# seung-lab/crackle

Measured on AMD Instinct MI355X. Metric: voxels/s encode+decode, 1024x1024x512 uint32; bit-exact .ckl bytes, higher is better.
Workload: dtype u32

## Files before the change

crackle_amd/csrc/ckl_trail.hpp:

```cpp
#pragma once

#include "ckl_device.hpp"

namespace ckl {
namespace dev {

constexpr uint32_t kTrailTileShift = 5, kTrailTileDim = 32;
__device__ __forceinline__ uint32_t mt_index(uint32_t mx, uint32_t my, uint32_t mtx2) {
	return (((my >> 1) * mtx2 + (mx >> 1)) << 2) | ((my & 1u) << 1) | (mx & 1u);
}
struct MicroTile {
	uint4 lo, hi;
	uint32_t mx, my;
	__device__ __forceinline__ bool holds(uint32_t x, uint32_t y) const { return (x >> 3) == mx && (y >> 3) == my; }
	__device__ __forceinline__ uint32_t nib(uint32_t x, uint32_t y) const {
		const uint32_t r = y & 7u;
		const uint32_t a0 = (r & 1u) ? lo.y : lo.x, a1 = (r & 1u) ? lo.w : lo.z, a2 = (r & 1u) ? hi.y : hi.x, a3 = (r & 1u) ? hi.w : hi.z;
		const uint32_t b0 = (r & 2u) ? a1 : a0, b1 = (r & 2u) ? a3 : a2;
		return (((r & 4u) ? b1 : b0) >> ((x & 7u) * 4u)) & 15u;
	}
};

enum : uint32_t { TRAIL_ERR_CAPACITY = 1u };
constexpr uint32_t kDartNone = 0xFFFFFFFFu;
// ... 532 lines not shown
			val = cm_load(j);
			if (val != ~0ull) {
				root = tuf_find<LDS>(parent, j);
				if (root == j) root = 0xFFFFFFFFu;
			}
		}
		unsigned long long todo = __ballot(root != 0xFFFFFFFFu);
		while (todo) {
			const int first = __ffsll(static_cast<long long>(todo)) - 1;
			const uint32_t r0 = __shfl(root, first, kWave);
			const bool mine = (root == r0);
			unsigned long long v = mine ? val : ~0ull;
#pragma unroll
			for (int s = kWave / 2; s >= 1; s >>= 1) {
				const unsigned long long o = __shfl_xor(v, s, kWave);
				v = o < v ? o : v;
			}
			if ((threadIdx.x & (kWave - 1)) == first) atomicMin(compmin + r0, v);
			todo &= ~__ballot(mine);
		}
	}
	__syncthreads();
	if (!CMLDS) __threadfence();
	stamp(13);
	uint32_t* bits = a.start_bits + static_cast<uint64_t>(zi) * a.start_words;
	for (uint32_t j = threadIdx.x; j < nn; j += kCompBlock) {
		if (tuf_load<LDS>(parent, j) != j) continue;
		const unsigned long long m = cm_load(j);
		if (m == ~0ull) continue;
		const uint32_t minv = static_cast<uint32_t>(m >> 32);
		const uint32_t d = static_cast<uint32_t>(m);
		const uint64_t db = nb * 4u;
		const uint32_t len = a.dart_len[db + d];
		const uint32_t mp = a.dart_minpos[db + d];
		const uint32_t d2 = a.dart_end[db + d];
		atomicOr(bits + (minv >> 5), 1u << (minv & 31u));
		{
			const uint32_t slot = atomicAdd(s_nstart, 1u);
			if (slot < kStartList) start_tmp[slot] = minv;
		}
		const uint32_t pos = mp >> 2, arr = mp & 3u;
		if (pos == 0 || pos == len) continue;
		const uint32_t s = atomicAdd(a.n_nodes + zi, 1u);
		if (s >= a.ncap[zi]) { atomicOr(a.slice_err + zi, TRAIL_ERR_CAPACITY); continue; }
		a.node_vertex[nb + s] = minv;
		a.node_adj[nb + s] = 5u;
		a.vert2node[static_cast<uint64_t>(zi) * a.nverts + minv] = s;
		const uint32_t other = arr ^ 2u;
		for (uint32_t q = 0; q < 4; q++) { a.dart_end[db + s * 4u + q] = kDartNone; a.dart_len[db + s * 4u + q] = 0; a.dart_inline[db + s * 4u + q] = 0; }
		a.dart_end[db + d] = (s << 2) | arr;        a.dart_len[db + d] = pos;
		a.dart_end[db + d2] = (s << 2) | other;     a.dart_len[db + d2] = len - pos;
		a.dart_end[db + s * 4u + arr] = d;          a.dart_len[db + s * 4u + arr] = pos;
		a.dart_end[db + s * 4u + other] = d2;       a.dart_len[db + s * 4u + other] = len - pos;
	}
	__syncthreads();
	if (LDS && CMLDS) __threadfence_block(); else __threadfence();
	stamp(14);
	uint32_t* starts = a.starts + nb;
	const uint32_t cap = a.kcap[zi];
	const uint32_t n_listed = *s_nstart;
	if (n_listed <= kStartList) {
		for (uint32_t i = threadIdx.x; i < n_listed; i += kCompBlock) {
			const uint32_t v = __hip_atomic_load(start_tmp + i, __ATOMIC_RELAXED, __HIP_MEMORY_SCOPE_AGENT);
			uint32_t rank = 0;
			for (uint32_t q = 0; q < n_listed; q++) rank += __hip_atomic_load(start_tmp + q, __ATOMIC_RELAXED, __HIP_MEMORY_SCOPE_AGENT) < v ? 1u : 0u;
			if (rank < cap) starts[rank] = v;
			else atomicOr(a.slice_err + zi, TRAIL_ERR_CAPACITY);
		}
		if (threadIdx.x == 0) a.n_starts[zi] = n_listed < cap ? n_listed : cap;
		stamp(15);
		return;
	}
	constexpr uint32_t kPer = 8;
	uint32_t carry = 0, err = 0;
	for (uint32_t w0 = 0; w0 < a.start_words; w0 += kCompBlock * kPer) {
		uint32_t b[kPer], cnt = 0;
#pragma unroll
		for (uint32_t q = 0; q < kPer; q++) {
			const uint32_t wi = w0 + threadIdx.x * kPer + q;
			b[q] = wi < a.start_words ? __hip_atomic_load(bits + wi, __ATOMIC_RELAXED, __HIP_MEMORY_SCOPE_AGENT) : 0u;
			cnt += __popc(b[q]);
		}
		uint32_t v[1] = { cnt }, tot[1];
		block_excl_add<1, kCompBlock / kWave>(v, tot, s_scan);
		uint32_t o = carry + v[0];
#pragma unroll
		for (uint32_t q = 0; q < kPer; q++) {
			const uint32_t wi = w0 + threadIdx.x * kPer + q;
			for (uint32_t m = b[q]; m; m &= m - 1u) {
				if (o < cap) starts[o] = wi * 32u + (__ffs(m) - 1);
				else err = TRAIL_ERR_CAPACITY;
				o++;
			}
		}
		carry += tot[0];
	}
	if (threadIdx.x == 0) a.n_starts[zi] = carry < cap ? carry : cap;
	if (err) atomicOr(a.slice_err + zi, err);
	stamp(15);
}

static __global__ void __launch_bounds__(kCompBlock) k_trail_components(TrailArgs a, uint32_t lds_bytes) {
	extern __shared__ unsigned long long s_comp[];
	__shared__ uint32_t s_scan[kCompBlock / kWave];
	__shared__ uint32_t s_nstart;
	const uint32_t zi = blockIdx.x + a.z0;
	const uint32_t nn = min(a.n_nodes[zi], a.ncap[zi]);
	if (threadIdx.x == 0) s_nstart = 0;
	__syncthreads();
	if (static_cast<uint64_t>(nn) * 12u <= lds_bytes) trail_components_slice<true, true>(a, zi, reinterpret_cast<uint32_t*>(s_comp + nn), s_comp, nn, s_scan, &s_nstart);
	else if (static_cast<uint64_t>(nn) * 4u <= lds_bytes) trail_components_slice<true, false>(a, zi, reinterpret_cast<uint32_t*>(s_comp), a.compmin + a.nbase[zi], nn, s_scan, &s_nstart);
	else trail_components_slice<false, false>(a, zi, a.parent + a.nbase[zi], a.compmin + a.nbase[zi], nn, s_scan, &s_nstart);
}

enum : uint32_t { TCODE_UP = 0, TCODE_RIGHT = 1, TCODE_DOWN = 2, TCODE_LEFT = 3, TCODE_NONE = 0xFE };

struct TrailTabLds {
	uint8_t* adj;
	unsigned long long* end4;
	__device__ __forceinline__ void load(uint32_t j, uint32_t& av, uint32_t& e_lo, uint32_t& e_hi) const {
		const uint32_t a0 = adj[j];
		const unsigned long long e = end4[j];
		av = __builtin_amdgcn_readfirstlane(a0);
		e_lo = __builtin_amdgcn_readfirstlane(static_cast<uint32_t>(e));
		e_hi = __builtin_amdgcn_readfirstlane(static_cast<uint32_t>(e >> 32));
	}
	__device__ __forceinline__ uint32_t pick(uint32_t e_lo, uint32_t e_hi, uint32_t k) const {
		const uint32_t w = (k & 2u) ? e_hi : e_lo;
		return (w >> ((k & 1u) * 16u)) & 0xFFFFu;
	}
	__device__ __forceinline__ void set_adj(uint32_t j, uint32_t v) const { adj[j] = static_cast<uint8_t>(v); }
};
struct TrailTabGlobal {
	uint8_t* adj;
	const uint32_t* end;
	__device__ __forceinline__ void load(uint32_t j, uint32_t& av, uint32_t& e_lo, uint32_t& e_hi) const {
		const uint32_t* w = reinterpret_cast<const uint32_t*>(reinterpret_cast<uintptr_t>(adj + j) & ~static_cast<uintptr_t>(3));
		const uint32_t sh = static_cast<uint32_t>(reinterpret_cast<uintptr_t>(adj + j) & 3u) * 8u;
		av = (__builtin_amdgcn_readfirstlane(__hip_atomic_load(w, __ATOMIC_RELAXED, __HIP_MEMORY_SCOPE_AGENT)) >> sh) & 0xFFu;
		e_lo = j; e_hi = 0;
	}
	__device__ __forceinline__ uint32_t pick(uint32_t e_lo, uint32_t e_hi, uint32_t k) const { return __builtin_amdgcn_readfirstlane(end[e_lo * 4u + k]); }
	__device__ __forceinline__ void set_adj(uint32_t j, uint32_t v) const {
		uint32_t* w = reinterpret_cast<uint32_t*>(reinterpret_cast<uintptr_t>(adj + j) & ~static_cast<uintptr_t>(3));
		const uint32_t sh = static_cast<uint32_t>(reinterpret_cast<uintptr_t>(adj + j) & 3u) * 8u;
		const uint32_t old = __hip_atomic_load(w, __ATOMIC_RELAXED, __HIP_MEMORY_SCOPE_AGENT);
		__hip_atomic_store(w, (old & ~(0xFFu << sh)) | ((v & 0xFFu) << sh), __ATOMIC_RELAXED, __HIP_MEMORY_SCOPE_AGENT);
	}
};

constexpr uint32_t kEvSeg = 0u << 30, kEvBseg = 1u << 30, kEvDead = 2u << 30, kEvEnd = 3u << 30, kEvMask = 3u << 30;
constexpr uint32_t kEvFormatAddr12 = 1u << 31;
constexpr uint32_t kEvWalkWide = 1u << 30;

template <typename TAB>
__device__ __forceinline__ void trail_walk_slice(
	const TrailArgs& a, uint32_t zi, const TAB& tab, uint2* s_stack2, uint32_t lds_slots
) {
	const uint64_t nb = a.nbase[zi];
	const uint32_t* starts = a.starts + nb;
	const uint32_t n_starts = a.n_starts[zi];
	uint32_t* ev = a.events + a.ibase[zi];
	const uint32_t ecap = a.icap[zi];
	uint32_t* st_node = a.stack_node + a.sbase[zi];
	uint32_t* st_ev = a.stack_item + a.sbase[zi];
	const uint32_t scap = a.scap[zi];
	uint32_t* ch_node = a.chain_node + a.kbase[zi];
	uint32_t* ch_ev0 = a.chain_ev0 + a.kbase[zi];
	const uint32_t kcap = a.kcap[zi];
	const uint32_t* vert2node = a.vert2node + static_cast<uint64_t>(zi) * a.nverts;
	const uint32_t cap1 = lds_slots - 1u;

	uint32_t ne = 0, nch = 0, err = 0;
	const unsigned long long dbg_t0 = (kTuning && a.dbg) ? __builtin_amdgcn_s_memtime() : 0ull;
	const unsigned long long dbg_r0 = (kTuning && a.dbg) ? __builtin_amdgcn_s_memrealtime() : 0ull;
	for (uint32_t si = 0; si < n_starts && !err; si++) {
		const uint32_t sv = __builtin_amdgcn_readfirstlane(starts[si]);
		uint32_t j = __builtin_amdgcn_readfirstlane(vert2node[sv]);
		if (nch < kcap) { ch_node[nch] = sv; ch_ev0[nch] = ne; }
		else err |= TRAIL_ERR_CAPACITY;
		nch++;
		uint32_t sp = 0, pend = 0;
		for (;;) {
			if (ne + 2u > ecap) { err |= TRAIL_ERR_CAPACITY; break; }
			uint32_t av_raw, e_lo, e_hi;
			tab.load(j, av_raw, e_lo, e_hi);
			const uint2 top = s_stack2[sp < cap1 ? sp : cap1];
			const uint32_t av = av_raw & ~pend;
			if (av == 0) {
				tab.set_adj(j, 0u);
				if (sp == 0) { ev[ne] = kEvEnd; ne++; break; }
				uint32_t pj = __builtin_amdgcn_readfirstlane(top.x), pev = __builtin_amdgcn_readfirstlane(top.y);
				if (sp > cap1) {
					pj = __builtin_amdgcn_readfirstlane(__hip_atomic_load(st_node + sp - 1u, __ATOMIC_RELAXED, __HIP_MEMORY_SCOPE_AGENT));
					pev = __builtin_amdgcn_readfirstlane(__hip_atomic_load(st_ev + sp - 1u, __ATOMIC_RELAXED, __HIP_MEMORY_SCOPE_AGENT));
				}
				ev[ne] = kEvDead | pev;
				ne++; sp--; pend = 0; j = pj;
				continue;
			}
			const uint32_t k = __ffs(av) - 1;
			const uint32_t rest = av & ~(1u << k);
			tab.set_adj(j, rest);
			const uint32_t e = tab.pick(e_lo, e_hi, k);
			const bool multi = rest != 0;
			if (multi && sp >= cap1) {
				if (sp < scap) { st_node[sp] = j; st_ev[sp] = ne; }
				else err |= TRAIL_ERR_CAPACITY;
			}
			s_stack2[(multi && sp < cap1) ? sp + 1u : 0u] = make_uint2(j, ne);
			ev[ne] = (multi ? kEvBseg : kEvSeg) | (j * 4u + k);
			ne++;
			sp += multi ? 1u : 0u;
			pend = 1u << (e & 3u);
			j = e >> 2;
		}
	}
	if (kTuning && a.dbg) {
		atomicAdd(a.dbg + 8, static_cast<unsigned long long>(ne));
		atomicAdd(a.dbg + 9, __builtin_amdgcn_s_memtime() - dbg_t0);
		atomicAdd(a.dbg + 10, __builtin_amdgcn_s_memrealtime() - dbg_r0);
		atomicAdd(a.dbg + 11, 1ull);
	}
	a.n_events[zi] = ne < ecap ? ne : ecap;
	a.n_chains[zi] = nch < kcap ? nch : kcap;
	if (err) atomicOr(a.slice_err + zi, err);
}

__device__ __forceinline__ uint32_t trail_walk_chain_fast(
	uint32_t j_addr, uint32_t& ev_off, uint32_t& ev_left, uint32_t stack_base, uint32_t max_depth, uint32_t* ev
) {
	uint32_t status, off = ev_off, left = ev_left;
	const uint32_t top0 = stack_base - 4u;
	const uint32_t ev_lo = __builtin_amdgcn_readfirstlane(static_cast<uint32_t>(reinterpret_cast<uintptr_t>(ev)));
	const uint32_t ev_hi = __builtin_amdgcn_readfirstlane(static_cast<uint32_t>(reinterpret_cast<uintptr_t>(ev) >> 32));
	j_addr = __builtin_amdgcn_readfirstlane(j_addr);
	max_depth = __builtin_amdgcn_readfirstlane(max_depth);
	asm volatile(
		"s_setprio 3\n"
		"s_mov_b32 s40, %[j]\n"
		"s_mov_b32 s41, 0\n"
		"s_mov_b32 s42, 0\n"
		"v_readfirstlane_b32 s43, %[left]\n"
		"s_mov_b32 s52, %[evlo]\n"
		"s_mov_b32 s53, %[evhi]\n"
		"s_mov_b32 s54, %[maxd]\n"
		"v_mov_b32 v29, %[off]\n"
		"v_mov_b32 v25, %[top]\n"
		"1:\n"
		"v_mov_b32 v20, s40\n"
		"ds_read2_b32 v[32:33], v20 offset1:1\n"
		"ds_read_b32 v34, v20 offset:8\n"
		"ds_read_b32 v26, v25\n"
		"s_sub_u32 s43, s43, 1\n"
		"s_cbranch_scc1 8f\n"
		"s_waitcnt lgkmcnt(0)\n"
		"v_readfirstlane_b32 s46, v32\n"
		"v_readfirstlane_b32 s44, v33\n"
		"v_readfirstlane_b32 s45, v34\n"
		"s_andn2_b32 s46, s46, s41\n"
		"s_cbranch_scc0 4f\n"
		"s_ff1_i32_b32 s47, s46\n"
		"s_bitset0_b32 s46, s47\n"
		"v_mov_b32 v21, s46\n"
		"ds_write_b32 v20, v21\n"
		"s_lshl_b32 s48, s47, 4\n"
		"s_lshr_b64 s[44:45], s[44:45], s48\n"
		"s_or_b32 s49, s40, s47\n"
		"s_cmp_eq_u32 s46, 0\n"
		"s_cbranch_scc1 3f\n"
		"s_cmp_ge_u32 s42, s54\n"
		"s_cbranch_scc1 9f\n"
		"s_bitset1_b32 s49, 30\n"
		"v_add_u32 v25, 4, v25\n"
		"v_lshl_or_b32 v28, v29, 14, s40\n"
		"s_add_u32 s42, s42, 1\n"
		"ds_write_b32 v25, v28\n"
		"3:\n"
		"v_mov_b32 v30, s49\n"
		"global_store_dword v29, v30, s[52:53]\n"
		"v_add_u32 v29, 4, v29\n"
		"s_and_b32 s48, s44, 3\n"
		"s_lshl_b32 s41, 1, s48\n"
		"s_and_b32 s40, s44, 0xfffc\n"
		"s_branch 1b\n"
		"4:\n"
		"v_mov_b32 v21, 0\n"
		"ds_write_b32 v20, v21\n"
		"s_cmp_eq_u32 s42, 0\n"
		"s_cbranch_scc1 7f\n"
		"v_readfirstlane_b32 s49, v26\n"
		"s_and_b32 s40, s49, 0xffff\n"
		"s_lshr_b32 s49, s49, 16\n"
		"s_bitset1_b32 s49, 31\n"
		"v_mov_b32 v30, s49\n"
		"global_store_dword v29, v30, s[52:53]\n"
		"v_add_u32 v29, 4, v29\n"
		"v_add_u32 v25, -4, v25\n"
		"s_sub_u32 s42, s42, 1\n"
		"s_mov_b32 s41, 0\n"
		"s_branch 1b\n"
		"7:\n"
		"v_mov_b32 v30, 0xc0000000\n"
		"global_store_dword v29, v30, s[52:53]\n"
		"v_add_u32 v29, 4, v29\n"
		"s_mov_b32 s48, 0\n"
// ... 105 lines not shown
		"s_cmp_eq_u32 s46, 0\n"
		"s_cbranch_scc1 3f\n"
		"s_cmp_ge_u32 s42, s54\n"
		"s_cbranch_scc1 9f\n"
		"s_bitset1_b32 s49, 30\n"
		"v_add_u32 v25, 4, v25\n"
		"v_lshl_or_b32 v28, v29, 12, s51\n"
		"s_add_u32 s42, s42, 1\n"
		"ds_write_b32 v25, v28\n"
		"3:\n"
		"v_mov_b32 v30, s49\n"
		"global_store_dword v29, v30, s[52:53]\n"
		"v_add_u32 v29, 4, v29\n"
		"s_and_b32 s48, s44, 3\n"
		"s_lshl_b32 s41, 1, s48\n"
		"s_and_b32 s40, s44, 0xfffc\n"
		"s_lshl_b32 s40, s40, 1\n"
		"s_branch 1b\n"
		"4:\n"
		"v_mov_b32 v21, 0\n"
		"ds_write_b8 v22, v21\n"
		"s_cmp_eq_u32 s42, 0\n"
		"s_cbranch_scc1 7f\n"
		"v_readfirstlane_b32 s49, v26\n"
		"s_and_b32 s40, s49, 0x3fff\n"
		"s_lshl_b32 s40, s40, 3\n"
		"s_lshr_b32 s49, s49, 14\n"
		"s_bitset1_b32 s49, 31\n"
		"v_mov_b32 v30, s49\n"
		"global_store_dword v29, v30, s[52:53]\n"
		"v_add_u32 v29, 4, v29\n"
		"v_add_u32 v25, -4, v25\n"
		"s_sub_u32 s42, s42, 1\n"
		"s_mov_b32 s41, 0\n"
		"s_branch 1b\n"
		"7:\n"
		"v_mov_b32 v30, 0xc0000000\n"
		"global_store_dword v29, v30, s[52:53]\n"
		"v_add_u32 v29, 4, v29\n"
		"s_mov_b32 s48, 0\n"
		"s_branch 6f\n"
		"8:\n"
		"s_mov_b32 s43, 0\n"
		"s_mov_b32 s48, 1\n"
		"s_branch 6f\n"
		"9:\n"
		"s_mov_b32 s48, 2\n"
		"6:\n"
		"s_setprio 0\n"
		"s_waitcnt lgkmcnt(0)\n"
		"v_mov_b32 %[off], v29\n"
		"v_mov_b32 %[left], s43\n"
		"v_mov_b32 %[st], s48\n"
		: [off] "+v"(off), [left] "+v"(left), [st] "=v"(status)
		: [j] "s"(j8), [top] "v"(top0), [evlo] "s"(ev_lo), [evhi] "s"(ev_hi), [maxd] "s"(max_depth), [adjb] "s"(adj_base)
		: "memory", "scc", "s40", "s41", "s42", "s43", "s44", "s45", "s46", "s47", "s48", "s49", "s50", "s51", "s52", "s53", "s54", "s55",
		  "v20", "v21", "v22", "v25", "v26", "v28", "v29", "v30", "v32", "v33", "v34");
	ev_off = __builtin_amdgcn_readfirstlane(off);
	ev_left = __builtin_amdgcn_readfirstlane(left);
	return __builtin_amdgcn_readfirstlane(status);
}

__device__ __forceinline__ bool trail_walk_slice_wide(const TrailArgs& a, uint32_t zi, uint32_t adj_base, uint32_t stack_base, uint32_t lds_bytes) {
	const uint64_t nb = a.nbase[zi];
	const uint32_t* starts = a.starts + nb;
	const uint32_t n_starts = a.n_starts[zi];
	uint32_t* ev = a.events + a.ibase[zi];
	const uint32_t ecap = a.icap[zi];
	uint32_t* ch_node = a.chain_node + a.kbase[zi];
	uint32_t* ch_ev0 = a.chain_ev0 + a.kbase[zi];
	const uint32_t kcap = a.kcap[zi];
	const uint32_t* vert2node = a.vert2node + static_cast<uint64_t>(zi) * a.nverts;
	const uint32_t max_depth = min((lds_bytes - stack_base) / 4u, a.walk_stack_cap);
	uint32_t off = 0, left = min(ecap, 262143u), nch = 0, err = 0;
	for (uint32_t si = 0; si < n_starts && !err; si++) {
		const uint32_t sv = __builtin_amdgcn_readfirstlane(starts[si]);
		const uint32_t j = __builtin_amdgcn_readfirstlane(vert2node[sv]);
		if (nch < kcap) { ch_node[nch] = sv; ch_ev0[nch] = off >> 2; }
		else err |= TRAIL_ERR_CAPACITY;
		nch++;
		const uint32_t st = trail_walk_chain_wide(j, off, left, adj_base, stack_base, max_depth, ev);
		if (st == 2u || (st == 1u && ecap > 262143u)) return false;
		if (st) err |= TRAIL_ERR_CAPACITY;
	}
	a.n_events[zi] = (off >> 2) | kEvWalkWide;
	a.n_chains[zi] = nch < kcap ? nch : kcap;
	if (err) atomicOr(a.slice_err + zi, err);
	return true;
}

constexpr uint32_t kWalkRegBlocks = 56, kWalkRegNodes = 64u * kWalkRegBlocks;
__device__ __forceinline__ uint32_t trail_walk_slice_regs_asm(
	uint32_t nblk, uint32_t list_base, uint32_t n_starts, uint32_t stack_base, uint32_t max_depth, uint32_t* ev, uint32_t* chain_ev0, uint32_t& ev_off, uint32_t& ev_left
) {
	uint32_t status, off = 0, left = ev_left;
	const uint32_t top0 = stack_base - 4u;
	const uint32_t ev_lo = __builtin_amdgcn_readfirstlane(static_cast<uint32_t>(reinterpret_cast<uintptr_t>(ev)));
	const uint32_t ev_hi = __builtin_amdgcn_readfirstlane(static_cast<uint32_t>(reinterpret_cast<uintptr_t>(ev) >> 32));
	const uint32_t c0_lo = __builtin_amdgcn_readfirstlane(static_cast<uint32_t>(reinterpret_cast<uintptr_t>(chain_ev0)));
	const uint32_t c0_hi = __builtin_amdgcn_readfirstlane(static_cast<uint32_t>(reinterpret_cast<uintptr_t>(chain_ev0) >> 32));
	nblk = __builtin_amdgcn_readfirstlane(nblk);
	list_base = __builtin_amdgcn_readfirstlane(list_base);
	n_starts = __builtin_amdgcn_readfirstlane(n_starts);
	max_depth = __builtin_amdgcn_readfirstlane(max_depth);
	asm volatile(
		"s_mov_b32 s61, m0\n"
		"s_mov_b64 s[62:63], exec\n"
		"s_mov_b64 exec, -1\n"
		"v_mbcnt_lo_u32_b32 v20, -1, 0\n"
		"v_mbcnt_hi_u32_b32 v20, -1, v20\n"
		"v_mul_u32_u24 v20, 12, v20\n"
		"s_mov_b32 s50, 0\n"
		"10:\n"
		"ds_read2_b32 v[32:33], v20 offset1:1\n"
		"ds_read_b32 v34, v20 offset:8\n"
		"s_waitcnt lgkmcnt(0)\n"
		"s_set_gpr_idx_on s50, gpr_idx(DST)\n"
		"s_nop 0\n"
		"v_mov_b32 v64, v32\n"
		"v_mov_b32 v120, v33\n"
		"v_mov_b32 v176, v34\n"
		"s_set_gpr_idx_off\n"
		"v_add_u32 v20, 0x300, v20\n"
		"s_add_u32 s50, s50, 1\n"
		"s_cmp_lt_u32 s50, %[nblk]\n"
		"s_cbranch_scc1 10b\n"
		"s_mov_b64 exec, 1\n"
		"s_setprio 3\n"
		"v_readfirstlane_b32 s43, %[left]\n"
		"s_mov_b32 s52, %[evlo]\n"
		"s_mov_b32 s53, %[evhi]\n"
		"s_mov_b32 s54, %[maxd]\n"
		"s_mov_b32 s58, %[c0lo]\n"
		"s_mov_b32 s59, %[c0hi]\n"
		"s_mov_b32 s56, %[nst]\n"
		"s_mov_b32 s57, %[list]\n"
		"s_mov_b32 s55, 0\n"
		"v_mov_b32 v29, 0\n"
		"20:\n"
		"s_cmp_ge_u32 s55, s56\n"
		"s_cbranch_scc1 30f\n"
		"s_lshl_b32 s48, s55, 2\n"
		"s_add_u32 s49, s48, s57\n"
		"v_mov_b32 v21, s49\n"
		"ds_read_b32 v21, v21\n"
		"v_lshrrev_b32 v22, 2, v29\n"
		"v_mov_b32 v24, s48\n"
		"global_store_dword v24, v22, s[58:59]\n"
		"s_mov_b32 s41, 0\n"
		"s_mov_b32 s42, 0\n"
		"v_mov_b32 v25, %[top]\n"
		"s_waitcnt lgkmcnt(0)\n"
		"v_readfirstlane_b32 s40, v21\n"
		"1:\n"
		"s_lshr_b32 s50, s40, 6\n"
		"s_and_b32 s51, s40, 63\n"
		"ds_read_b32 v26, v25\n"
		"s_set_gpr_idx_on s50, gpr_idx(SRC0)\n"
		"s_nop 0\n"
		"v_readlane_b32 s46, v64, s51\n"
		"v_readlane_b32 s44, v120, s51\n"
		"v_readlane_b32 s45, v176, s51\n"
		"s_set_gpr_idx_off\n"
		"s_sub_u32 s43, s43, 1\n"
		"s_cbranch_scc1 8f\n"
		"s_andn2_b32 s46, s46, s41\n"
		"s_cbranch_scc0 4f\n"
		"s_ff1_i32_b32 s47, s46\n"
		"s_bitset0_b32 s46, s47\n"
		"s_lshl_b64 exec, 1, s51\n"
		"s_set_gpr_idx_on s50, gpr_idx(DST)\n"
		"s_nop 0\n"
		"v_mov_b32 v64, s46\n"
		"s_set_gpr_idx_off\n"
		"s_mov_b64 exec, 1\n"
		"s_lshl_b32 s48, s47, 4\n"
		"s_lshr_b64 s[44:45], s[44:45], s48\n"
		"s_lshl_b32 s49, s40, 2\n"
		"s_or_b32 s49, s49, s47\n"
		"s_cmp_eq_u32 s46, 0\n"
		"s_cbranch_scc1 3f\n"
		"s_cmp_ge_u32 s42, s54\n"
		"s_cbranch_scc1 9f\n"
		"s_bitset1_b32 s49, 30\n"
		"v_add_u32 v25, 4, v25\n"
		"v_lshl_or_b32 v28, v29, 12, s40\n"
		"s_add_u32 s42, s42, 1\n"
		"ds_write_b32 v25, v28\n"
		"3:\n"
		"v_mov_b32 v30, s49\n"
		"global_store_dword v29, v30, s[52:53]\n"
		"v_add_u32 v29, 4, v29\n"
		"s_and_b32 s48, s44, 3\n"
		"s_lshl_b32 s41, 1, s48\n"
		"s_bfe_u32 s40, s44, 0xe0002\n"
		"s_branch 1b\n"
		"4:\n"
		"s_lshl_b64 exec, 1, s51\n"
		"s_set_gpr_idx_on s50, gpr_idx(DST)\n"
		"s_nop 0\n"
		"v_mov_b32 v64, 0\n"
		"s_set_gpr_idx_off\n"
		"s_mov_b64 exec, 1\n"
		"s_cmp_eq_u32 s42, 0\n"
		"s_cbranch_scc1 7f\n"
		"s_waitcnt lgkmcnt(0)\n"
		"v_readfirstlane_b32 s49, v26\n"
		"s_and_b32 s40, s49, 0x3fff\n"
		"s_lshr_b32 s49, s49, 14\n"
		"s_bitset1_b32 s49, 31\n"
		"v_mov_b32 v30, s49\n"
		"global_store_dword v29, v30, s[52:53]\n"
		"v_add_u32 v29, 4, v29\n"
		"v_add_u32 v25, -4, v25\n"
		"s_sub_u32 s42, s42, 1\n"
		"s_mov_b32 s41, 0\n"
		"s_branch 1b\n"
		"7:\n"
		"v_mov_b32 v30, 0xc0000000\n"
		"global_store_dword v29, v30, s[52:53]\n"
		"v_add_u32 v29, 4, v29\n"
		"s_add_u32 s55, s55, 1\n"
		"s_branch 20b\n"
		"30:\n"
		"s_mov_b32 s48, 0\n"
		"s_branch 6f\n"
		"8:\n"
		"s_mov_b32 s43, 0\n"
		"s_mov_b32 s48, 1\n"
		"s_branch 6f\n"
		"9:\n"
		"s_mov_b32 s48, 2\n"
		"6:\n"
		"s_setprio 0\n"
		"s_waitcnt lgkmcnt(0)\n"
		"s_mov_b64 exec, s[62:63]\n"
		"s_mov_b32 m0, s61\n"
		"v_readfirstlane_b32 s49, v29\n"
		"v_mov_b32 %[off], s49\n"
		"v_mov_b32 %[left], s43\n"
		"v_mov_b32 %[st], s48\n"
		: [off] "+v"(off), [left] "+v"(left), [st] "=v"(status)
		: [nblk] "s"(nblk), [list] "s"(list_base), [nst] "s"(n_starts), [top] "v"(top0), [evlo] "s"(ev_lo), [evhi] "s"(ev_hi), [c0lo] "s"(c0_lo), [c0hi] "s"(c0_hi), [maxd] "s"(max_depth)
		: "memory", "scc", "s40", "s41", "s42", "s43", "s44", "s45", "s46", "s47", "s48", "s49", "s50", "s51", "s52", "s53", "s54", "s55", "s56", "s57", "s58", "s59", "s61", "s62", "s63",
		  "v20", "v21", "v22", "v24", "v25", "v26", "v28", "v29", "v30", "v32", "v33", "v34",
		  "v64", "v65", "v66", "v67", "v68", "v69", "v70", "v71", "v72", "v73", "v74", "v75", "v76", "v77", "v78", "v79", "v80", "v81", "v82", "v83", "v84", "v85", "v86", "v87", "v88", "v89", "v90", "v91", "v92", "v93", "v94", "v95", "v96", "v97", "v98", "v99", "v100", "v101", "v102", "v103", "v104", "v105", "v106", "v107", "v108", "v109", "v110", "v111", "v112", "v113", "v114", "v115", "v116", "v117", "v118", "v119", "v120", "v121", "v122", "v123", "v124", "v125", "v126", "v127", "v128", "v129", "v130", "v131", "v132", "v133", "v134", "v135", "v136", "v137", "v138", "v139", "v140", "v141", "v142", "v143", "v144", "v145", "v146", "v147", "v148", "v149", "v150", "v151", "v152", "v153", "v154", "v155", "v156", "v157", "v158", "v159", "v160", "v161", "v162", "v163", "v164", "v165", "v166", "v167", "v168", "v169", "v170", "v171", "v172", "v173", "v174", "v175", "v176", "v177", "v178", "v179", "v180", "v181", "v182", "v183", "v184", "v185", "v186", "v187", "v188", "v189", "v190", "v191", "v192", "v193", "v194", "v195", "v196", "v197", "v198", "v199", "v200", "v201", "v202", "v203", "v204", "v205", "v206", "v207", "v208", "v209", "v210", "v211", "v212", "v213", "v214", "v215", "v216", "v217", "v218", "v219", "v220", "v221", "v222", "v223", "v224", "v225", "v226", "v227", "v228", "v229", "v230", "v231");
	ev_off = __builtin_amdgcn_readfirstlane(off);
	ev_left = __builtin_amdgcn_readfirstlane(left);
	return __builtin_amdgcn_readfirstlane(status);
}

static __global__ void __launch_bounds__(kWave) k_trail_walk(TrailArgs a, uint32_t lds_bytes) {
	extern __shared__ uint32_t s_trail[];
	const uint32_t zi = blockIdx.x + a.z0;
	const uint32_t nn = min(a.n_nodes[zi], a.ncap[zi]);
	const uint64_t nb = a.nbase[zi];
	if (a.slice_err[zi]) {
		if (threadIdx.x == 0) { a.n_events[zi] = 0; a.n_chains[zi] = 0; }
		return;
	}
	const unsigned long long dbg_k0 = (kTuning && a.dbg) ? __builtin_amdgcn_s_memtime() : 0ull;
	if (!a.walk_plain && !a.walk_no_regs && nn <= kWalkRegNodes && __builtin_amdgcn_readfirstlane(static_cast<uint32_t>(reinterpret_cast<uintptr_t>(s_trail))) == 0u) {
		const uint32_t nblk = (nn + 63u) / 64u;
		const uint32_t recs = nblk * 64u * 12u;
		const uint32_t n_starts = a.n_starts[zi];
		const uint32_t list_bytes = ((n_starts * 4u + 15u) / 16u) * 16u;
		const uint32_t kcap = a.kcap[zi];
		const uint32_t ecap = a.icap[zi];
		if (nblk > 0u && n_starts <= kcap && recs + list_bytes + 2048u <= lds_bytes) {
			for (uint32_t j = threadIdx.x; j < nblk * 64u; j += kWave) {
				uint32_t e[4] = { 0xFFFFu, 0xFFFFu, 0xFFFFu, 0xFFFFu };
				if (j < nn) {
#pragma unroll
					for (uint32_t k = 0; k < 4; k++) {
						const uint32_t d = a.dart_end[(nb + j) * 4u + k];
						e[k] = d == kDartNone ? 0xFFFFu : d;
					}
				}
				s_trail[j * 3u] = j < nn ? a.node_adj[nb + j] : 0u;
				s_trail[j * 3u + 1u] = e[0] | (e[1] << 16);
				s_trail[j * 3u + 2u] = e[2] | (e[3] << 16);
			}
			const uint32_t* starts = a.starts + nb;
			const uint32_t* vert2node = a.vert2node + static_cast<uint64_t>(zi) * a.nverts;
			uint32_t* ch_node = a.chain_node + a.kbase[zi];
			for (uint32_t si = threadIdx.x; si < n_starts; si += kWave) {
				const uint32_t sv = starts[si];
				s_trail[recs / 4u + si] = vert2node[sv];
				ch_node[si] = sv;
			}
			__syncthreads();
			const uint32_t stack_base = recs + list_bytes;
			const uint32_t max_depth = min((lds_bytes - stack_base) / 4u, a.walk_stack_cap);
			uint32_t off = 0, left = min(ecap, 262143u);
			const uint32_t st = trail_walk_slice_regs_asm(nblk, recs, n_starts, stack_base, max_depth, a.events + a.ibase[zi], a.chain_ev0 + a.kbase[zi], off, left);
			if (st == 0u || (st == 1u && ecap <= 262143u)) {
				if (threadIdx.x == 0) {
					a.n_events[zi] = (off >> 2) | kEvWalkWide;
					a.n_chains[zi] = n_starts;
					if (st) atomicOr(a.slice_err + zi, TRAIL_ERR_CAPACITY);
				}
				return;
			}
			__syncthreads();
		}
	}
	const uint32_t rec_bytes = nn * 12u + 16u;
	if (!a.walk_plain && nn < 5461u && rec_bytes + 2048u <= lds_bytes && __builtin_amdgcn_readfirstlane(static_cast<uint32_t>(reinterpret_cast<uintptr_t>(s_trail))) == 0u) {
		for (uint32_t j = threadIdx.x; j < nn; j += kWave) {
			uint32_t e[4];
#pragma unroll
			for (uint32_t k = 0; k < 4; k++) {
				const uint32_t d = a.dart_end[(nb + j) * 4u + k];
				e[k] = d == kDartNone ? 0xFFFFu : (((d >> 2) * 12u) | (d & 3u));
			}
			s_trail[j * 3u] = a.node_adj[nb + j];
			s_trail[j * 3u + 1u] = e[0] | (e[1] << 16);
			s_trail[j * 3u + 2u] = e[2] | (e[3] << 16);
		}
		__syncthreads();
		if (kTuning && a.dbg && threadIdx.x == 0) atomicAdd(a.dbg + 6, __builtin_amdgcn_s_memtime() - dbg_k0);
		bool done = false;
		if (threadIdx.x == 0) done = trail_walk_slice_fast(a, zi, rec_bytes, lds_bytes);
		if (kTuning && a.dbg && threadIdx.x == 0) atomicAdd(a.dbg + 7, __builtin_amdgcn_s_memtime() - dbg_k0);
		if (__builtin_amdgcn_readfirstlane(done ? 1u : 0u)) return;
		__syncthreads();
	}
	const uint32_t tab_bytes = ((nn * 9u + 15u) / 16u) * 16u;
	const bool in_lds = nn < 16384u && tab_bytes + 2048u <= lds_bytes;
	if (in_lds) {
		TrailTabLds t;
		t.end4 = reinterpret_cast<unsigned long long*>(s_trail);
		t.adj = reinterpret_cast<uint8_t*>(s_trail) + nn * 8u;
		uint16_t* e16 = reinterpret_cast<uint16_t*>(s_trail);
		auto fill = [&]() {
			for (uint32_t d = threadIdx.x; d < nn * 4u; d += kWave) {
				const uint32_t e = a.dart_end[nb * 4u + d];
				e16[d] = static_cast<uint16_t>(e == kDartNone ? 0xFFFFu : e);
			}
			for (uint32_t j = threadIdx.x; j < nn; j += kWave) t.adj[j] = a.node_adj[nb + j];
			__syncthreads();
		};
		fill();
		if (!a.walk_plain && tab_bytes + 2048u <= lds_bytes && __builtin_amdgcn_readfirstlane(static_cast<uint32_t>(reinterpret_cast<uintptr_t>(s_trail))) == 0u) {
			bool done = false;
			if (threadIdx.x == 0) done = trail_walk_slice_wide(a, zi, nn * 8u, tab_bytes, lds_bytes);
			if (__builtin_amdgcn_readfirstlane(done ? 1u : 0u)) return;
			__syncthreads();
			fill();
		}
		if (threadIdx.x == 0) trail_walk_slice<TrailTabLds>(a, zi, t, reinterpret_cast<uint2*>(s_trail + tab_bytes / 4u), (lds_bytes - tab_bytes) / 8u);
	}
	else if (threadIdx.x == 0) {
		TrailTabGlobal t;
		t.adj = a.node_adj + nb;
		t.end = a.dart_end + nb * 4u;
		trail_walk_slice<TrailTabGlobal>(a, zi, t, reinterpret_cast<uint2*>(s_trail), lds_bytes / 8u);
	}
}

constexpr uint32_t kXiRib = 1u << 31, kXiDead = 1u << 30, kXiPrevDead = 1u << 29, kXiMask = (1u << 29) - 1u;

struct TrailEvents {
	const uint32_t* ev;
	const int32_t* lnp;
	uint32_t n;
	__device__ __forceinline__ bool first(uint32_t i) const { return i == 0 || (ev[i - 1] & kEvMask) == kEvEnd; }
	__device__ __forceinline__ int32_t rib_of(uint32_t i) const {
		if ((ev[i] & kEvMask) != kEvDead || i == 0) return -1;
		const int32_t q = lnp[i - 1];
		if (q < 0 || (ev[q] & kEvMask) != kEvBseg || !first(static_cast<uint32_t>(q))) return -1;
		return q;
	}
	__device__ __forceinline__ bool dead(uint32_t i) const {
		const uint32_t k = ev[i] & kEvMask;
		return k == kEvEnd || (k == kEvDead && rib_of(i) < 0);
	}
};

constexpr int kItemsBlock = 1024;

static __global__ void __launch_bounds__(kItemsBlock) k_trail_items(TrailArgs a) {
	constexpr int kNW = kItemsBlock / kWave;
	__shared__ uint32_t s_scan[kNW];
	__shared__ int32_t s_scan_max[kNW];
	const uint32_t zi = blockIdx.x + a.z0;
	if (a.slice_err[zi]) {
		if (threadIdx.x == 0) a.n_items[zi] = 0;
		return;
	}
	const uint32_t n = a.n_events[zi] & ~(kEvFormatAddr12 | kEvWalkWide);
	const bool addr12 = (a.n_events[zi] & kEvFormatAddr12) != 0;
	auto dart = [&](uint32_t e) -> uint32_t {
		const uint32_t p = e & ~kEvMask;
		return addr12 ? (((((p >> 2) * 0xAAABu) >> 17) << 2) | (p & 3u)) : p;
	};
	const uint64_t ib = a.ibase[zi], nb = a.nbase[zi];
	const uint32_t* ev = a.events + ib;
	int32_t* lnp = reinterpret_cast<int32_t*>(a.item_off + ib);
	int32_t* lnd = reinterpret_cast<int32_t*>(a.ev_lnd + ib);
	uint32_t* xi = a.ev_item + ib;
	uint32_t* items = a.items + ib;
	const uint32_t icap = a.icap[zi];
	const uint32_t* dend = a.dart_end + nb * 4u;
	constexpr uint32_t kPer = 4;
	constexpr uint32_t kNone = 4u, kLeft = 1u, kUp = 3u;
	constexpr uint32_t kB = kItemCtl | TCODE_UP | (TCODE_DOWN << 2), kBalt = kItemCtl | TCODE_LEFT | (TCODE_RIGHT << 2);
	constexpr uint32_t kT = kItemCtl | TCODE_DOWN | (TCODE_UP << 2), kTalt = kItemCtl | TCODE_RIGHT | (TCODE_LEFT << 2);

	{
		int32_t carry = -1;
		for (uint32_t i0 = 0; i0 < n; i0 += kItemsBlock * kPer) {
			int32_t v[kPer], run = -1;
#pragma unroll
			for (uint32_t q = 0; q < kPer; q++) {
				const uint32_t i = i0 + threadIdx.x * kPer + q;
				if (i < n && (ev[i] & kEvMask) != kEvSeg) run = static_cast<int32_t>(i);
				v[q] = run;
			}
			int32_t total;
			const int32_t excl = block_excl_max<kNW>(run, total, s_scan_max);
			const int32_t pre = carry > excl ? carry : excl;
#pragma unroll
			for (uint32_t q = 0; q < kPer; q++) {
				const uint32_t i = i0 + threadIdx.x * kPer + q;
				if (i < n) lnp[i] = v[q] > pre ? v[q] : pre;
			}
			carry = carry > total ? carry : total;
		}
	}
	__syncthreads();
	__threadfence_block();
	TrailEvents te = { ev, lnp, n };

	uint32_t total_items = 0;
	{
		int32_t carry_max = -1;
		for (uint32_t i0 = 0; i0 < n; i0 += kItemsBlock * kPer) {
			uint32_t cnt[kPer], fl[kPer], sum = 0;
			int32_t v[kPer], run = -1;
#pragma unroll
			for (uint32_t q = 0; q < kPer; q++) {
				const uint32_t i = i0 + threadIdx.x * kPer + q;
				cnt[q] = 0; fl[q] = 0;
				if (i < n) {
					const uint32_t k = ev[i] & kEvMask;
					if (k == kEvSeg) cnt[q] = 1;
					else if (k == kEvBseg) cnt[q] = 2;
					else {
						const bool rib = k == kEvDead && te.rib_of(i) >= 0;
						const bool prev_dead = !te.first(i) && te.dead(i - 1);
						if (rib) fl[q] = kXiRib;
						else { fl[q] = kXiDead | (prev_dead ? kXiPrevDead : 0u); cnt[q] = prev_dead ? 0u : 1u; }
					}
					if (!(fl[q] & kXiDead)) run = static_cast<int32_t>(i);
				}
				v[q] = run;
				sum += cnt[q];
			}
			uint32_t sv[1] = { sum }, tot[1];
			block_excl_add<1, kNW>(sv, tot, s_scan);
			int32_t total_max;
			const int32_t excl = block_excl_max<kNW>(run, total_max, s_scan_max);
			const int32_t pre = carry_max > excl ? carry_max : excl;
			uint32_t x = total_items + sv[0];
#pragma unroll
			for (uint32_t q = 0; q < kPer; q++) {
				const uint32_t i = i0 + threadIdx.x * kPer + q;
				if (i < n) {
					xi[i] = x | fl[q];
					lnd[i] = v[q] > pre ? v[q] : pre;
				}
				x += cnt[q];
			}
			total_items += tot[0];
			carry_max = carry_max > total_max ? carry_max : total_max;
		}
	}
	__syncthreads();
	__threadfence_block();
	if (total_items > icap || total_items > kXiMask) {
		if (threadIdx.x == 0) { atomicOr(a.slice_err + zi, TRAIL_ERR_CAPACITY); a.n_items[zi] = 0; }
		return;
	}

	auto last_simple = [&](uint32_t i) -> uint32_t {
		if (te.first(i)) return kNone;
		const uint32_t p = ev[i - 1];
		if ((p & kEvMask) == kEvDead) {
			const int32_t q = lnp[i - 2];
			return (ev[q] & 3u) ^ 1u;
		}
		return (dend[dart(p)] & 3u) ^ 1u;
	};
	auto last_before = [&](uint32_t i) -> uint32_t {
		if (te.first(i) || !(xi[i - 1] & kXiDead)) return last_simple(i);
		const uint32_t r = static_cast<uint32_t>(lnd[i - 1] + 1);
		const uint32_t lb = last_simple(r);
		return ((0x18u >> lb) & 1u) ? kLeft : kUp;
	};

	for (uint32_t i = threadIdx.x; i < n; i += kItemsBlock) {
		const uint32_t e = ev[i], k = e & kEvMask, xf = xi[i], x = xf & kXiMask;
		if (k == kEvSeg) items[x] = kItemSeg | dart(e);
		else if (k == kEvBseg) {
			const uint32_t lb = last_before(i);
			items[x] = ((0x14u >> lb) & 1u) ? kBalt : kB;
			items[x + 1] = kItemSeg | dart(e);
		}
		else if ((xf & (kXiDead | kXiPrevDead)) == kXiDead) {
			const uint32_t lb = last_simple(i);
			items[x] = ((0x18u >> lb) & 1u) ? kTalt : kT;
		}
	}
	__syncthreads();
	__threadfence_block();

	for (uint32_t i = threadIdx.x; i < n; i += kItemsBlock) {
		const uint32_t xf = xi[i];
		if ((xf & (kXiDead | kXiPrevDead)) == (kXiDead | kXiPrevDead)) {
			const uint32_t b = ev[i - 1] & ~kEvMask;
			items[xi[b] & kXiMask] = kItemDead;
		}
		if (xf & kXiRib) {
			const uint32_t q = static_cast<uint32_t>(lnp[i - 1]);
			const uint32_t x0 = xi[q] & kXiMask;
			items[x0] = kItemDead;
			const uint32_t* ev0 = a.chain_ev0 + a.kbase[zi];
			uint32_t lo = 0, hi = a.n_chains[zi];
			while (hi - lo > 1u) { const uint32_t mid = (lo + hi) >> 1; if (ev0[mid] <= q) lo = mid; else hi = mid; }
			a.chain_node[a.kbase[zi] + lo] = a.node_vertex[nb + (dend[dart(ev[i - 1])] >> 2)];
			for (uint32_t m = q; m < i; m++) items[x0 + 1u + (i - 1u - m)] = kItemSeg | dend[dart(ev[m])];
		}
	}
	__syncthreads();
	{
		const uint32_t nch = a.n_chains[zi];
		const uint32_t* ev0 = a.chain_ev0 + a.kbase[zi];
		uint32_t* item0 = a.chain_item0 + a.kbase[zi];
		for (uint32_t c = threadIdx.x; c < nch; c += kItemsBlock) item0[c] = ev0[c] < n ? (xi[ev0[c]] & kXiMask) : total_items;
	}
	if (threadIdx.x == 0) a.n_items[zi] = total_items;
}

static __global__ void __launch_bounds__(kBlock) k_trail_offsets(TrailArgs a) {
	__shared__ uint32_t s_scan[kWaves];
	const uint32_t zi = blockIdx.x + a.z0;
	const uint32_t n = a.n_items[zi];
	const uint32_t* items = a.items + a.ibase[zi];
	uint32_t* off = a.item_off + a.ibase[zi];
	const uint32_t* dlen = a.dart_len + a.nbase[zi] * 4u;
	constexpr uint32_t kPer = 4;
	uint32_t carry = 0;
	for (uint32_t i0 = 0; i0 < n; i0 += kBlock * kPer) {
		uint32_t len[kPer], cnt = 0;
#pragma unroll
		for (uint32_t q = 0; q < kPer; q++) {
			const uint32_t i = i0 + threadIdx.x * kPer + q;
			len[q] = 0;
			if (i < n) {
				const uint32_t it = items[i];
				const uint32_t kind = it & kItemMask;
				len[q] = kind == kItemSeg ? dlen[it & ~kItemMask] : (kind == kItemCtl ? 2u : 0u);
			}
			cnt += len[q];
		}
		uint32_t v[1] = { cnt }, tot[1];
		block_excl_add<1>(v, tot, s_scan);
		uint32_t o = carry + v[0];
#pragma unroll
		for (uint32_t q = 0; q < kPer; q++) {
			const uint32_t i = i0 + threadIdx.x * kPer + q;
			if (i < n) off[i] = o;
			o += len[q];
		}
		carry += tot[0];
	}
	__syncthreads();
	__threadfence_block();
	const uint32_t total = carry;
	const uint32_t nch = a.n_chains[zi];
	const uint32_t* item0 = a.chain_item0 + a.kbase[zi];
	uint32_t* ch_off = a.chain_off + a.kbase[zi];
	uint32_t* ch_clen = a.chain_clen + a.kbase[zi];
	for (uint32_t c = threadIdx.x; c < nch; c += kBlock) {
		const uint32_t o0 = item0[c] < n ? off[item0[c]] : total;
		const uint32_t o1 = (c + 1 < nch && item0[c + 1] < n) ? off[item0[c + 1]] : total;
		ch_off[c] = o0;
		ch_clen[c] = o1 - o0;
	}
	if (threadIdx.x == 0) {
		a.n_raw[zi] = total;
		a.n_valid[zi] = total;
		if (total > a.ccap[zi]) atomicOr(a.slice_err + zi, TRAIL_ERR_CAPACITY);
	}
}

static __global__ void __launch_bounds__(kBlock) k_trail_expand(TrailArgs a) {
	__shared__ uint32_t s_long[kWaves][kExpandChunk];
	const uint32_t zi = blockIdx.y + a.z0;
	if (a.slice_err[zi]) return;
	const uint32_t lane = threadIdx.x & (kWave - 1);
	const uint32_t wv = threadIdx.x >> 6;
	const uint32_t wave = blockIdx.x * kWaves + wv;
	const uint32_t n_items = a.n_items[zi];
	const uint32_t range_begin = wave * kExpandChunk;
	const uint32_t range_end = min(range_begin + kExpandChunk, n_items);
	if (range_begin >= range_end) return;
	const uint64_t nb = a.nbase[zi];
	const uint32_t* items = a.items + a.ibase[zi];
	const uint32_t* item_off = a.item_off + a.ibase[zi];
	uint8_t* cp0 = a.cp + a.cbase[zi];
	const uint4* adjm = a.adjm + zi * a.adjm_stride;
	const unsigned long long lt_mask = (1ull << lane) - 1ull;
	uint32_t* longs = s_long[wv];
	struct __attribute__((packed)) U64 { unsigned long long v; };
	struct __attribute__((packed)) U32 { uint32_t v; };
	struct __attribute__((packed)) U16 { uint16_t v; };
	auto store_tail = [](uint8_t* o, unsigned long long v, uint32_t n) {
		if (n & 4u) { reinterpret_cast<U32*>(o)->v = static_cast<uint32_t>(v); o += 4; v >>= 32; }
		if (n & 2u) { reinterpret_cast<U16*>(o)->v = static_cast<uint16_t>(v); o += 2; v >>= 16; }
		if (n & 1u) o[0] = static_cast<uint8_t>(v);
	};

	uint32_t n_long = 0;
	for (uint32_t i0 = range_begin; i0 < range_end; i0 += kWave) {
		const uint32_t i = i0 + lane;
		bool walk = false;
		if (i < range_end) {
			const uint32_t it = items[i], kind = it & kItemMask;
			uint8_t* o = cp0 + item_off[i];
			if (kind == kItemCtl) reinterpret_cast<U16*>(o)->v = static_cast<uint16_t>((it & 3u) | (((it >> 2) & 3u) << 8));
			else if (kind == kItemSeg) {
				const uint32_t d = it & ~kItemMask;
				const uint32_t len = a.dart_len[nb * 4u + d];
				if (len && a.dart_inline[nb * 4u + d] && len <= kInlineCodes) {
					const uint4 q = a.dart_codes[nb * 4u + d];
					const uint32_t w[4] = { q.x, q.y, q.z, q.w };
#pragma unroll
					for (uint32_t g = 0; g < kInlineCodes / 8u; g++) {
						if (g * 8u < len) {
							const uint32_t h = (w[g >> 1] >> ((g & 1u) * 16u)) & 0xFFFFu;
							uint32_t lo = h & 0xFFu, hi = h >> 8;
							lo = (lo | (lo << 12)) & 0x000F000Fu; lo = (lo | (lo << 6)) & 0x03030303u;
// ... 66 lines not shown
```

Measured before the change: 161.1 billion.

## Re-encode register-resident trail records to trim the asm walk inner loop

Changes the packed per-node record used by the register-resident trail walker. Adjacency bits now sit shifted by 6 with the lane index in the low bits, and dart ends are stored as a 12-bit node plus a one-hot direction bit. This lets the inline-asm walk use v_writelane with a self-indexed lane and drop the exec-mask juggling and one readlane per step, and the dead-end path is restructured into its own loop. A new event format flag tells the items kernel to subtract a bias when decoding darts. The change also adds timing probes that are compiled out unless tuning is enabled, and the new encoding must stay bit-exact across kernels.

```diff
diff --git a/crackle_amd/csrc/ckl_trail.hpp b/crackle_amd/csrc/ckl_trail.hpp
--- a/crackle_amd/csrc/ckl_trail.hpp
+++ b/crackle_amd/csrc/ckl_trail.hpp
@@ -708,6 +708,7 @@
 constexpr uint32_t kEvSeg = 0u << 30, kEvBseg = 1u << 30, kEvDead = 2u << 30, kEvEnd = 3u << 30, kEvMask = 3u << 30;
 constexpr uint32_t kEvFormatAddr12 = 1u << 31;
 constexpr uint32_t kEvWalkWide = 1u << 30;
+constexpr uint32_t kEvFormatRegs = kEvFormatAddr12 | kEvWalkWide;
 
 template <typename TAB>
 __device__ __forceinline__ void trail_walk_slice(
@@ -1119,34 +1120,58 @@
 		"v_mov_b32 v25, %[top]\n"
 		"s_waitcnt lgkmcnt(0)\n"
 		"v_readfirstlane_b32 s40, v21\n"
+		"s_nop 3\n"
+		"s_branch 1f\n"
+		"4:\n"
+		"v_writelane_b32 v64, s46, s46\n"
+		"s_set_gpr_idx_off\n"
+		"5:\n"
+		"s_cmp_eq_u32 s42, 0\n"
+		"s_cbranch_scc1 7f\n"
+		"s_waitcnt lgkmcnt(0)\n"
+		"v_readfirstlane_b32 s49, v26\n"
+		"v_add_u32 v25, -4, v25\n"
+		"s_and_b32 s40, s49, 0x3fff\n"
+		"s_lshr_b32 s49, s49, 14\n"
+		"s_bitset1_b32 s49, 31\n"
+		"v_mov_b32 v30, s49\n"
+		"global_store_dword v29, v30, s[52:53]\n"
+		"v_add_u32 v29, 4, v29\n"
+		"s_sub_u32 s42, s42, 1\n"
+		"s_lshr_b32 s50, s40, 6\n"
+		"ds_read_b32 v26, v25\n"
+		"s_set_gpr_idx_on s50, gpr_idx(SRC0,DST)\n"
+		"s_nop 0\n"
+		"v_readlane_b32 s46, v64, s40\n"
+		"s_sub_u32 s43, s43, 1\n"
+		"s_cbranch_scc1 8f\n"
+		"s_and_b32 s47, s46, 0x3c0\n"
+		"s_cbranch_scc1 2f\n"
+		"s_set_gpr_idx_off\n"
+		"s_branch 5b\n"
 		"1:\n"
 		"s_lshr_b32 s50, s40, 6\n"
-		"s_and_b32 s51, s40, 63\n"
 		"ds_read_b32 v26, v25\n"
-		"s_set_gpr_idx_on s50, gpr_idx(SRC0)\n"
+		"s_set_gpr_idx_on s50, gpr_idx(SRC0,DST)\n"
 		"s_nop 0\n"
-		"v_readlane_b32 s46, v64, s51\n"
-		"v_readlane_b32 s44, v120, s51\n"
-		"v_readlane_b32 s45, v176, s51\n"
-		"s_set_gpr_idx_off\n"
+		"v_readlane_b32 s46, v64, s40\n"
 		"s_sub_u32 s43, s43, 1\n"
 		"s_cbranch_scc1 8f\n"
 		"s_andn2_b32 s46, s46, s41\n"
-		"s_cbranch_scc0 4f\n"
-		"s_ff1_i32_b32 s47, s46\n"
+		"s_and_b32 s47, s46, 0x3c0\n"
+		"s_cbranch_scc0 4b\n"
+		"2:\n"
+		"v_readlane_b32 s45, v120, s40\n"
+		"v_readlane_b32 s44, v176, s40\n"
+		"s_ff1_i32_b32 s47, s47\n"
 		"s_bitset0_b32 s46, s47\n"
-		"s_lshl_b64 exec, 1, s51\n"
-		"s_set_gpr_idx_on s50, gpr_idx(DST)\n"
-		"s_nop 0\n"
-		"v_mov_b32 v64, s46\n"
+		"v_writelane_b32 v64, s46, s46\n"
 		"s_set_gpr_idx_off\n"
-		"s_mov_b64 exec, 1\n"
 		"s_lshl_b32 s48, s47, 4\n"
 		"s_lshr_b64 s[44:45], s[44:45], s48\n"
-		"s_lshl_b32 s49, s40, 2\n"
-		"s_or_b32 s49, s49, s47\n"
-		"s_cmp_eq_u32 s46, 0\n"
-		"s_cbranch_scc1 3f\n"
+		"s_lshl2_add_u32 s49, s40, s47\n"
+		"s_and_b32 s48, s46, 0x3c0\n"
+		"s_cbranch_scc0 3f\n"
 		"s_cmp_ge_u32 s42, s54\n"
 		"s_cbranch_scc1 9f\n"
 		"s_bitset1_b32 s49, 30\n"
@@ -1158,30 +1183,9 @@
 		"v_mov_b32 v30, s49\n"
 		"global_store_dword v29, v30, s[52:53]\n"
 		"v_add_u32 v29, 4, v29\n"
-		"s_and_b32 s48, s44, 3\n"
-		"s_lshl_b32 s41, 1, s48\n"
-		"s_bfe_u32 s40, s44, 0xe0002\n"
-		"s_branch 1b\n"
-		"4:\n"
-		"s_lshl_b64 exec, 1, s51\n"
-		"s_set_gpr_idx_on s50, gpr_idx(DST)\n"
-		"s_nop 0\n"
-		"v_mov_b32 v64, 0\n"
-		"s_set_gpr_idx_off\n"
-		"s_mov_b64 exec, 1\n"
-		"s_cmp_eq_u32 s42, 0\n"
-		"s_cbranch_scc1 7f\n"
-		"s_waitcnt lgkmcnt(0)\n"
-		"v_readfirstlane_b32 s49, v26\n"
-		"s_and_b32 s40, s49, 0x3fff\n"
-		"s_lshr_b32 s49, s49, 14\n"
-		"s_bitset1_b32 s49, 31\n"
-		"v_mov_b32 v30, s49\n"
-		"global_store_dword v29, v30, s[52:53]\n"
-		"v_add_u32 v29, 4, v29\n"
-		"v_add_u32 v25, -4, v25\n"
-		"s_sub_u32 s42, s42, 1\n"
-		"s_mov_b32 s41, 0\n"
+		"s_lshr_b32 s41, s44, 6\n"
+		"s_and_b32 s41, s41, 0x3c0\n"
+		"s_and_b32 s40, s44, 0xfff\n"
 		"s_branch 1b\n"
 		"7:\n"
 		"v_mov_b32 v30, 0xc0000000\n"
@@ -1193,6 +1197,7 @@
 		"s_mov_b32 s48, 0\n"
 		"s_branch 6f\n"
 		"8:\n"
+		"s_set_gpr_idx_off\n"
 		"s_mov_b32 s43, 0\n"
 		"s_mov_b32 s48, 1\n"
 		"s_branch 6f\n"
@@ -1209,7 +1214,7 @@
 		"v_mov_b32 %[st], s48\n"
 		: [off] "+v"(off), [left] "+v"(left), [st] "=v"(status)
 		: [nblk] "s"(nblk), [list] "s"(list_base), [nst] "s"(n_starts), [top] "v"(top0), [evlo] "s"(ev_lo), [evhi] "s"(ev_hi), [c0lo] "s"(c0_lo), [c0hi] "s"(c0_hi), [maxd] "s"(max_depth)
-		: "memory", "scc", "s40", "s41", "s42", "s43", "s44", "s45", "s46", "s47", "s48", "s49", "s50", "s51", "s52", "s53", "s54", "s55", "s56", "s57", "s58", "s59", "s61", "s62", "s63",
+		: "memory", "scc", "s40", "s41", "s42", "s43", "s44", "s45", "s46", "s47", "s48", "s49", "s50", "s52", "s53", "s54", "s55", "s56", "s57", "s58", "s59", "s61", "s62", "s63",
 		  "v20", "v21", "v22", "v24", "v25", "v26", "v28", "v29", "v30", "v32", "v33", "v34",
 		  "v64", "v65", "v66", "v67", "v68", "v69", "v70", "v71", "v72", "v73", "v74", "v75", "v76", "v77", "v78", "v79", "v80", "v81", "v82", "v83", "v84", "v85", "v86", "v87", "v88", "v89", "v90", "v91", "v92", "v93", "v94", "v95", "v96", "v97", "v98", "v99", "v100", "v101", "v102", "v103", "v104", "v105", "v106", "v107", "v108", "v109", "v110", "v111", "v112", "v113", "v114", "v115", "v116", "v117", "v118", "v119", "v120", "v121", "v122", "v123", "v124", "v125", "v126", "v127", "v128", "v129", "v130", "v131", "v132", "v133", "v134", "v135", "v136", "v137", "v138", "v139", "v140", "v141", "v142", "v143", "v144", "v145", "v146", "v147", "v148", "v149", "v150", "v151", "v152", "v153", "v154", "v155", "v156", "v157", "v158", "v159", "v160", "v161", "v162", "v163", "v164", "v165", "v166", "v167", "v168", "v169", "v170", "v171", "v172", "v173", "v174", "v175", "v176", "v177", "v178", "v179", "v180", "v181", "v182", "v183", "v184", "v185", "v186", "v187", "v188", "v189", "v190", "v191", "v192", "v193", "v194", "v195", "v196", "v197", "v198", "v199", "v200", "v201", "v202", "v203", "v204", "v205", "v206", "v207", "v208", "v209", "v210", "v211", "v212", "v213", "v214", "v215", "v216", "v217", "v218", "v219", "v220", "v221", "v222", "v223", "v224", "v225", "v226", "v227", "v228", "v229", "v230", "v231");
 	ev_off = __builtin_amdgcn_readfirstlane(off);
@@ -1241,10 +1246,10 @@
 #pragma unroll
 					for (uint32_t k = 0; k < 4; k++) {
 						const uint32_t d = a.dart_end[(nb + j) * 4u + k];
-						e[k] = d == kDartNone ? 0xFFFFu : d;
+						e[k] = d == kDartNone ? 0xFFFFu : (((d >> 2) & 0xFFFu) | (0x1000u << (d & 3u)));
 					}
 				}
-				s_trail[j * 3u] = j < nn ? a.node_adj[nb + j] : 0u;
+				s_trail[j * 3u] = ((j < nn ? a.node_adj[nb + j] & 15u : 0u) << 6) | (j & 63u);
 				s_trail[j * 3u + 1u] = e[0] | (e[1] << 16);
 				s_trail[j * 3u + 2u] = e[2] | (e[3] << 16);
 			}
@@ -1260,10 +1265,20 @@
 			const uint32_t stack_base = recs + list_bytes;
 			const uint32_t max_depth = min((lds_bytes - stack_base) / 4u, a.walk_stack_cap);
 			uint32_t off = 0, left = min(ecap, 262143u);
+			const unsigned long long dbg_t0 = (kTuning && a.dbg) ? __builtin_amdgcn_s_memtime() : 0ull;
+			const unsigned long long dbg_r0 = (kTuning && a.dbg) ? __builtin_amdgcn_s_memrealtime() : 0ull;
 			const uint32_t st = trail_walk_slice_regs_asm(nblk, recs, n_starts, stack_base, max_depth, a.events + a.ibase[zi], a.chain_ev0 + a.kbase[zi], off, left);
+			if (kTuning && a.dbg && threadIdx.x == 0) {
+				atomicAdd(a.dbg + 6, dbg_t0 - dbg_k0);
+				atomicAdd(a.dbg + 7, __builtin_amdgcn_s_memtime() - dbg_k0);
+				atomicAdd(a.dbg + 8, static_cast<unsigned long long>(off >> 2));
+				atomicAdd(a.dbg + 9, __builtin_amdgcn_s_memtime() - dbg_t0);
+				atomicAdd(a.dbg + 10, __builtin_amdgcn_s_memrealtime() - dbg_r0);
+				atomicAdd(a.dbg + 11, 1ull);
+			}
 			if (st == 0u || (st == 1u && ecap <= 262143u)) {
 				if (threadIdx.x == 0) {
-					a.n_events[zi] = (off >> 2) | kEvWalkWide;
+					a.n_events[zi] = (off >> 2) | kEvFormatRegs;
 					a.n_chains[zi] = n_starts;
 					if (st) atomicOr(a.slice_err + zi, TRAIL_ERR_CAPACITY);
 				}
@@ -1357,10 +1372,11 @@
 		return;
 	}
 	const uint32_t n = a.n_events[zi] & ~(kEvFormatAddr12 | kEvWalkWide);
-	const bool addr12 = (a.n_events[zi] & kEvFormatAddr12) != 0;
+	const bool addr12 = (a.n_events[zi] & kEvFormatRegs) == kEvFormatAddr12;
+	const uint32_t dart_bias = (a.n_events[zi] & kEvFormatRegs) == kEvFormatRegs ? 6u : 0u;
 	auto dart = [&](uint32_t e) -> uint32_t {
 		const uint32_t p = e & ~kEvMask;
-		return addr12 ? (((((p >> 2) * 0xAAABu) >> 17) << 2) | (p & 3u)) : p;
+		return addr12 ? (((((p >> 2) * 0xAAABu) >> 17) << 2) | (p & 3u)) : p - dart_bias;
 	};
 	const uint64_t ib = a.ibase[zi], nb = a.nbase[zi];
 	const uint32_t* ev = a.events + ib;
@@ -1456,7 +1472,7 @@
 		const uint32_t p = ev[i - 1];
 		if ((p & kEvMask) == kEvDead) {
 			const int32_t q = lnp[i - 2];
-			return (ev[q] & 3u) ^ 1u;
+			return (dart(ev[q]) & 3u) ^ 1u;
 		}
 		return (dend[dart(p)] & 3u) ^ 1u;
 	};
```

After: 161.8 billion, median of 5. No clear change (+0.4%).
